# zacz08/ADM

Measured on AMD Instinct MI355X. Metric: train images/sec (CIFAR-10 32x32 uncond DDM UNet, 1 optimizer step/iter) + 10-step sample images/sec, higher is better.
Workload: dtype f32; 1 GPU; BASELINE configs[1]: CIFAR-10 32x32 uncond two-decoder DhariwalUNet (216M params), bs=128/GPU fp32, ddm_const schedule, dropout 0.1, loss_simple (LPIPS term needs unfetchable VGG16 weights), clip 1.0 + AdamW + EMA(every 8); global_batch=128, image=3x32x32, parallelism=dp1, valid=True

## Files before the change

### adm_amd/csrc/attention_h3.hip

```cpp
#include "common.h"
#include "split_format.h"

namespace {

constexpr int AH_KROW = 72;

__device__ __forceinline__ int ah_acc_row(int r, int lh) { return (r & 3) + 8 * (r >> 2) + 4 * lh; }
__device__ __forceinline__ int ah_pos16(int k) { return (((k >> 2) & 1) << 3) | ((k >> 3) << 2) | (k & 3); }

template <int NKT, bool MULTI>
__global__ __launch_bounds__(64 * NKT) void attn_fwd_h3_kernel(const float* __restrict__ qkv, float* __restrict__ out,
                                                                float* __restrict__ lse, int L, int heads,
                                                                const float* __restrict__ amax) {
  extern __shared__ __attribute__((aligned(16))) unsigned short smh[];
  constexpr int CH = NKT * 32;
  constexpr int VROW = CH + 8;
  unsigned short* Kh = smh;
  unsigned short* Vt = smh + 2 * CH * AH_KROW;
  const int tid = threadIdx.x, lane = tid & 63, wid = tid >> 6, lr = lane & 31, lh = lane >> 5;
  const int b = blockIdx.x / heads, h = blockIdx.x % heads;
  const long rs = (long)heads * 192;
  const float* base = qkv + (long)b * L * rs + h * 192;
  const float sc = split_scale(adm_amax_read(amax));
  const int q = (MULTI ? (int)blockIdx.y * CH : 0) + wid * 32 + lr;
  u32x4 q0[4], q1[4];
  {
    const float* qrow = base + (long)q * rs;
#pragma unroll
    for (int c = 0; c < 4; ++c) {
      const f32x4 lo = *reinterpret_cast<const f32x4*>(qrow + 16 * c + 8 * lh);
      const f32x4 hi = *reinterpret_cast<const f32x4*>(qrow + 16 * c + 8 * lh + 4);
      const float v[8] = {lo[0], lo[1], lo[2], lo[3], hi[0], hi[1], hi[2], hi[3]};
      split2_oct(v, sc * 0.125f, q0[c], q1[c]);
    }
  }
  const float inv_s = 1.f / (sc * sc);
  float m = -INFINITY, l = 0.f;
  f32x16 o[2];
#pragma unroll
  for (int r = 0; r < 16; ++r) { o[0][r] = 0.f; o[1][r] = 0.f; }
  const int nchunks = MULTI ? L / CH : 1;
#pragma unroll 1
  for (int kc = 0; kc < nchunks; ++kc) {
  const float* kbase = base + (long)kc * CH * rs;
  if (MULTI) __syncthreads();
  for (int i = tid; i < CH * 16; i += 64 * NKT) {
    const int key = i >> 4, c4 = i & 15;
    const f32x4 v = *reinterpret_cast<const f32x4*>(kbase + (long)key * rs + 64 + c4 * 4);
    unsigned t0[2], t1[2];
#pragma unroll
    for (int j = 0; j < 2; ++j) {
      const float x0 = v[2 * j] * sc, x1 = v[2 * j + 1] * sc;
      const _Float16 h00 = (_Float16)x0, h01 = (_Float16)x1;
      t0[j] = __builtin_bit_cast(unsigned, f16x2{h00, h01});
      t1[j] = __builtin_bit_cast(unsigned, f16x2{(_Float16)(x0 - (float)h00), (_Float16)(x1 - (float)h01)});
    }
    *reinterpret_cast<uint2*>(Kh + key * AH_KROW + c4 * 4) = make_uint2(t0[0], t0[1]);
    *reinterpret_cast<uint2*>(Kh + (CH + key) * AH_KROW + c4 * 4) = make_uint2(t1[0], t1[1]);
  }
  for (int i = tid; i < (CH / 2) * 16; i += 64 * NKT) {
    const int kp = i >> 4, c4 = i & 15;
    const int grp = kp >> 3, p0 = (kp & 7) * 2;
    const int k0 = grp * 16 + ((p0 & 7) & 3) + 8 * ((p0 & 7) >> 2) + 4 * (p0 >> 3);
    const f32x4 va = *reinterpret_cast<const f32x4*>(kbase + (long)k0 * rs + 128 + c4 * 4);
    const f32x4 vb = *reinterpret_cast<const f32x4*>(kbase + (long)(k0 + 1) * rs + 128 + c4 * 4);
#pragma unroll
    for (int j = 0; j < 4; ++j) {
      const float x0 = va[j] * sc, x1 = vb[j] * sc;
      const _Float16 h00 = (_Float16)x0, h01 = (_Float16)x1;
      const int d = c4 * 4 + j;
      *reinterpret_cast<unsigned*>(Vt + d * VROW + grp * 16 + p0) = __builtin_bit_cast(unsigned, f16x2{h00, h01});
      *reinterpret_cast<unsigned*>(Vt + (64 + d) * VROW + grp * 16 + p0) =
          __builtin_bit_cast(unsigned, f16x2{(_Float16)(x0 - (float)h00), (_Float16)(x1 - (float)h01)});
    }
  }
  __syncthreads();
  f32x16 s[NKT];
  float mc = -INFINITY;
#pragma unroll
  for (int kt = 0; kt < NKT; ++kt) {
    f32x16 acc;
#pragma unroll
    for (int r = 0; r < 16; ++r) acc[r] = 0.f;
    const unsigned short* krow = Kh + (kt * 32 + lr) * AH_KROW + 8 * lh;
#pragma unroll
    for (int c = 0; c < 4; ++c) {
      const f16x8 a0 = __builtin_bit_cast(f16x8, *reinterpret_cast<const u32x4*>(krow + 16 * c));
      const f16x8 a1 = __builtin_bit_cast(f16x8, *reinterpret_cast<const u32x4*>(krow + CH * AH_KROW + 16 * c));
      const f16x8 b0 = __builtin_bit_cast(f16x8, q0[c]), b1 = __builtin_bit_cast(f16x8, q1[c]);
      acc = __builtin_amdgcn_mfma_f32_32x32x16_f16(a0, b1, acc, 0, 0, 0);
      acc = __builtin_amdgcn_mfma_f32_32x32x16_f16(a1, b0, acc, 0, 0, 0);
      acc = __builtin_amdgcn_mfma_f32_32x32x16_f16(a0, b0, acc, 0, 0, 0);
    }
#pragma unroll
    for (int r = 0; r < 16; ++r) {
      s[kt][r] = acc[r] * inv_s;
      mc = fmaxf(mc, s[kt][r]);
    }
  }
  mc = fmaxf(mc, __shfl_xor(mc, 32, 64));
  const float mn = fmaxf(m, mc);
  if constexpr (MULTI) {
    const float rsc = (m == -INFINITY) ? 0.f : __expf(m - mn);
    l *= rsc;
#pragma unroll
    for (int r = 0; r < 16; ++r) { o[0][r] *= rsc; o[1][r] *= rsc; }
  }
#pragma unroll
  for (int kt = 0; kt < NKT; ++kt)
#pragma unroll
    for (int r = 0; r < 16; ++r) {
      const float e = __expf(s[kt][r] - mn);
      s[kt][r] = e;
      l += e;
    }
  m = mn;
#pragma unroll
  for (int kt = 0; kt < NKT; ++kt)
#pragma unroll
    for (int sl = 0; sl < 2; ++sl) {
      const float pv[8] = {s[kt][8 * sl], s[kt][8 * sl + 1], s[kt][8 * sl + 2], s[kt][8 * sl + 3],
                           s[kt][8 * sl + 4], s[kt][8 * sl + 5], s[kt][8 * sl + 6], s[kt][8 * sl + 7]};
      u32x4 p0, p1;
      split2_oct(pv, 16384.f, p0, p1);
      const f16x8 b0 = __builtin_bit_cast(f16x8, p0), b1 = __builtin_bit_cast(f16x8, p1);
#pragma unroll
      for (int db = 0; db < 2; ++db) {
        const unsigned short* vrow = Vt + (db * 32 + lr) * VROW + kt * 32 + 16 * sl + 8 * lh;
        const f16x8 a0 = __builtin_bit_cast(f16x8, *reinterpret_cast<const u32x4*>(vrow));
        const f16x8 a1 = __builtin_bit_cast(f16x8, *reinterpret_cast<const u32x4*>(vrow + 64 * VROW));
        o[db] = __builtin_amdgcn_mfma_f32_32x32x16_f16(a0, b1, o[db], 0, 0, 0);
        o[db] = __builtin_amdgcn_mfma_f32_32x32x16_f16(a1, b0, o[db], 0, 0, 0);
        o[db] = __builtin_amdgcn_mfma_f32_32x32x16_f16(a0, b0, o[db], 0, 0, 0);
      }
    }
  }
  const float mc = m;
  l += __shfl_xor(l, 32, 64);
  const float oscale = 1.f / (l * sc * 16384.f);
  float* orow = out + ((long)b * L + q) * heads * 64 + h * 64;
#pragma unroll
  for (int db = 0; db < 2; ++db)
#pragma unroll
    for (int q4 = 0; q4 < 4; ++q4) {
      const f32x4 v = {o[db][4 * q4] * oscale, o[db][4 * q4 + 1] * oscale, o[db][4 * q4 + 2] * oscale, o[db][4 * q4 + 3] * oscale};
      *reinterpret_cast<f32x4*>(orow + db * 32 + 8 * q4 + 4 * lh) = v;
    }
  if (lh == 0 && lse) lse[((long)b * heads + h) * L + q] = mc + __logf(l);
}

template <int NKT, bool MULTI>
int launch_fwd_h3(const float* qkv, float* out, float* lse, const float* amax, int B, int L, int heads, hipStream_t st) {
  constexpr int CH = NKT * 32;
  constexpr int smem = (2 * CH * AH_KROW + 2 * 64 * (CH + 8)) * (int)sizeof(unsigned short);
  static bool attr_set = false;
  if (!attr_set) {
    if (hipFuncSetAttribute(reinterpret_cast<const void*>(&attn_fwd_h3_kernel<NKT, MULTI>), hipFuncAttributeMaxDynamicSharedMemorySize, smem) != hipSuccess)
      return ADM_ELAUNCH;
    attr_set = true;
  }
  hipLaunchKernelGGL((attn_fwd_h3_kernel<NKT, MULTI>), dim3(B * heads, MULTI ? L / CH : 1), dim3(64 * NKT), smem, st, qkv, out, lse, L, heads, amax);
  ADM_CHECK_LAUNCH();
  return ADM_OK;
}

__device__ __forceinline__ f32x16 ah_mfma3(const u32x4 a0, const u32x4 a1, const u32x4 b0, const u32x4 b1, f32x16 c) {
  c = __builtin_amdgcn_mfma_f32_32x32x16_f16(__builtin_bit_cast(f16x8, a0), __builtin_bit_cast(f16x8, b1), c, 0, 0, 0);
  c = __builtin_amdgcn_mfma_f32_32x32x16_f16(__builtin_bit_cast(f16x8, a1), __builtin_bit_cast(f16x8, b0), c, 0, 0, 0);
  return __builtin_amdgcn_mfma_f32_32x32x16_f16(__builtin_bit_cast(f16x8, a0), __builtin_bit_cast(f16x8, b0), c, 0, 0, 0);
}
__device__ __forceinline__ void ah_fill_rows(unsigned short* dst, int CH, const float* src, long rs, float scale, int tid, int nthreads) {
  for (int i = tid; i < CH * 16; i += nthreads) {
    const int row = i >> 4, c4 = i & 15;
    const f32x4 v = *reinterpret_cast<const f32x4*>(src + (long)row * rs + c4 * 4);
    unsigned t0[2], t1[2];
#pragma unroll
    for (int j = 0; j < 2; ++j) {
      const float x0 = v[2 * j] * scale, x1 = v[2 * j + 1] * scale;
      const _Float16 h00 = (_Float16)x0, h01 = (_Float16)x1;
      t0[j] = __builtin_bit_cast(unsigned, f16x2{h00, h01});
      t1[j] = __builtin_bit_cast(unsigned, f16x2{(_Float16)(x0 - (float)h00), (_Float16)(x1 - (float)h01)});
    }
    *reinterpret_cast<uint2*>(dst + row * AH_KROW + c4 * 4) = make_uint2(t0[0], t0[1]);
    *reinterpret_cast<uint2*>(dst + (CH + row) * AH_KROW + c4 * 4) = make_uint2(t1[0], t1[1]);
  }
}
__device__ __forceinline__ void ah_fill_both(unsigned short* rimg, unsigned short* timg, int CH, const float* src, long rs, float scale,
                                             int tid, int nthreads) {
  const int VROW = CH + 8;
  for (int i = tid; i < (CH / 2) * 16; i += nthreads) {
    const int kp = i >> 4, c4 = i & 15;
    const int grp = kp >> 3, p0 = (kp & 7) * 2;
    const int r0 = grp * 16 + ((p0 & 7) & 3) + 8 * ((p0 & 7) >> 2) + 4 * (p0 >> 3);
    const f32x4 va = *reinterpret_cast<const f32x4*>(src + (long)r0 * rs + c4 * 4);
    const f32x4 vb = *reinterpret_cast<const f32x4*>(src + (long)(r0 + 1) * rs + c4 * 4);
    _Float16 a0[4], a1[4], b0[4], b1[4];
#pragma unroll
    for (int j = 0; j < 4; ++j) {
      const float x0 = va[j] * scale, x1 = vb[j] * scale;
      a0[j] = (_Float16)x0; a1[j] = (_Float16)(x0 - (float)a0[j]);
      b0[j] = (_Float16)x1; b1[j] = (_Float16)(x1 - (float)b0[j]);
      const int d = c4 * 4 + j;
      *reinterpret_cast<unsigned*>(timg + d * VROW + grp * 16 + p0) = __builtin_bit_cast(unsigned, f16x2{a0[j], b0[j]});
      *reinterpret_cast<unsigned*>(timg + (64 + d) * VROW + grp * 16 + p0) = __builtin_bit_cast(unsigned, f16x2{a1[j], b1[j]});
    }
    *reinterpret_cast<uint2*>(rimg + r0 * AH_KROW + c4 * 4) =
        make_uint2(__builtin_bit_cast(unsigned, f16x2{a0[0], a0[1]}), __builtin_bit_cast(unsigned, f16x2{a0[2], a0[3]}));
    *reinterpret_cast<uint2*>(rimg + (CH + r0) * AH_KROW + c4 * 4) =
        make_uint2(__builtin_bit_cast(unsigned, f16x2{a1[0], a1[1]}), __builtin_bit_cast(unsigned, f16x2{a1[2], a1[3]}));
    *reinterpret_cast<uint2*>(rimg + (r0 + 1) * AH_KROW + c4 * 4) =
        make_uint2(__builtin_bit_cast(unsigned, f16x2{b0[0], b0[1]}), __builtin_bit_cast(unsigned, f16x2{b0[2], b0[3]}));
    *reinterpret_cast<uint2*>(rimg + (CH + r0 + 1) * AH_KROW + c4 * 4) =
        make_uint2(__builtin_bit_cast(unsigned, f16x2{b1[0], b1[1]}), __builtin_bit_cast(unsigned, f16x2{b1[2], b1[3]}));
  }
}
__device__ __forceinline__ void ah_row_frag(const float* row, int lh, float scale, u32x4 (&t0)[4], u32x4 (&t1)[4]) {
#pragma unroll
  for (int c = 0; c < 4; ++c) {
    const f32x4 lo = *reinterpret_cast<const f32x4*>(row + 16 * c + 8 * lh);
    const f32x4 hi = *reinterpret_cast<const f32x4*>(row + 16 * c + 8 * lh + 4);
    const float v[8] = {lo[0], lo[1], lo[2], lo[3], hi[0], hi[1], hi[2], hi[3]};
    split2_oct(v, scale, t0[c], t1[c]);
  }
}
__device__ __forceinline__ f32x16 ah_rows_times_frag(const unsigned short* img, int CH, int row0, const u32x4 (&f0)[4], const u32x4 (&f1)[4],
                                                     int lr, int lh) {
  f32x16 acc;
#pragma unroll
  for (int r = 0; r < 16; ++r) acc[r] = 0.f;
  const unsigned short* rp = img + (row0 + lr) * AH_KROW + 8 * lh;
#pragma unroll
  for (int c = 0; c < 4; ++c)
    acc = ah_mfma3(*reinterpret_cast<const u32x4*>(rp + 16 * c), *reinterpret_cast<const u32x4*>(rp + CH * AH_KROW + 16 * c), f0[c], f1[c], acc);
  return acc;
}
__device__ __forceinline__ void ah_accum_T(f32x16 (&o)[2], const unsigned short* timg, int CH, int row0, const f32x16& t, float scale, int lr, int lh) {
  const int VROW = CH + 8;
#pragma unroll
  for (int sl = 0; sl < 2; ++sl) {
    const float tv[8] = {t[8 * sl], t[8 * sl + 1], t[8 * sl + 2], t[8 * sl + 3], t[8 * sl + 4], t[8 * sl + 5], t[8 * sl + 6], t[8 * sl + 7]};
    u32x4 b0, b1;
    split2_oct(tv, scale, b0, b1);
#pragma unroll
    for (int db = 0; db < 2; ++db) {
      const unsigned short* vp = timg + (db * 32 + lr) * VROW + row0 + 16 * sl + 8 * lh;
      o[db] = ah_mfma3(*reinterpret_cast<const u32x4*>(vp), *reinterpret_cast<const u32x4*>(vp + 64 * VROW), b0, b1, o[db]);
    }
  }
}
__device__ __forceinline__ void ah_store_T(const f32x16 (&o)[2], float* rowptr, int lh, float scale, float& am) {
#pragma unroll
  for (int db = 0; db < 2; ++db)
#pragma unroll
    for (int q4 = 0; q4 < 4; ++q4) {
      const f32x4 v = {o[db][4 * q4] * scale, o[db][4 * q4 + 1] * scale, o[db][4 * q4 + 2] * scale, o[db][4 * q4 + 3] * scale};
      am = fmaxf(fmaxf(am, fmaxf(fabsf(v[0]), fabsf(v[1]))), fmaxf(fabsf(v[2]), fabsf(v[3])));
      *reinterpret_cast<f32x4*>(rowptr + db * 32 + 8 * q4 + 4 * lh) = v;
    }
}

template <int NW>
__global__ __launch_bounds__(64 * NW) void attn_bwd_dq_h3_kernel(const float* __restrict__ qkv, const float* __restrict__ out,
                                                                   const float* __restrict__ dout, const float* __restrict__ lse,
                                                                   float* __restrict__ dqkv, float* __restrict__ delta, int L, int heads,
                                                                   const float* __restrict__ amax_qkv, const float* __restrict__ amax_g,
                                                                   float* __restrict__ amax_out) {
  extern __shared__ __attribute__((aligned(16))) unsigned short smh[];
  constexpr int CH = NW >= 4 ? 128 : 32 * NW;
  unsigned short* Kh = smh;
  unsigned short* Vh = Kh + 2 * CH * AH_KROW;
  unsigned short* Kt = Vh + 2 * CH * AH_KROW;
  const int tid = threadIdx.x, lane = tid & 63, wid = tid >> 6, lr = lane & 31, lh = lane >> 5;
  const int b = blockIdx.x / heads, h = blockIdx.x % heads;
  const long rs = (long)heads * 192, ro = (long)heads * 64;
  const float* base = qkv + (long)b * L * rs + h * 192;
  const float aq = adm_amax_read(amax_qkv), ag = adm_amax_read(amax_g);
  const float sc = split_scale(aq), sg = split_scale(ag), sd = split_scale(128.f * aq * ag);
  const int q = (int)blockIdx.y * 32 * NW + wid * 32 + lr;
  u32x4 q0[4], q1[4], g0[4], g1[4];
  ah_row_frag(base + (long)q * rs, lh, sc * 0.125f, q0, q1);
  const float* grow = dout + ((long)b * L + q) * ro + h * 64;
  const float* orow = out + ((long)b * L + q) * ro + h * 64;
  ah_row_frag(grow, lh, sg, g0, g1);
  float dl = 0.f;
#pragma unroll
  for (int c = 0; c < 4; ++c)
#pragma unroll
    for (int hh = 0; hh < 2; ++hh) {
      const f32x4 gv = *reinterpret_cast<const f32x4*>(grow + 16 * c + 8 * lh + 4 * hh);
      const f32x4 ov = *reinterpret_cast<const f32x4*>(orow + 16 * c + 8 * lh + 4 * hh);
      dl += gv[0] * ov[0] + gv[1] * ov[1] + gv[2] * ov[2] + gv[3] * ov[3];
    }
  dl += __shfl_xor(dl, 32, 64);
  const float ls = lse[((long)b * heads + h) * L + q];
  if (lh == 0) delta[((long)b * heads + h) * L + q] = dl;
  const float inv_s = 1.f / (sc * sc), inv_g = 1.f / (sc * sg);
  f32x16 dq[2];
#pragma unroll
  for (int r = 0; r < 16; ++r) { dq[0][r] = 0.f; dq[1][r] = 0.f; }
#pragma unroll 1
  for (int k0 = 0; k0 < L; k0 += CH) {
    __syncthreads();
    ah_fill_both(Kh, Kt, CH, base + (long)k0 * rs + 64, rs, sc, tid, 64 * NW);
    ah_fill_rows(Vh, CH, base + (long)k0 * rs + 128, rs, sc, tid, 64 * NW);
    __syncthreads();
#pragma unroll 1
    for (int kt = 0; kt < CH / 32; ++kt) {
      f32x16 s = ah_rows_times_frag(Kh, CH, kt * 32, q0, q1, lr, lh);
      const f32x16 dp = ah_rows_times_frag(Vh, CH, kt * 32, g0, g1, lr, lh);
#pragma unroll
      for (int r = 0; r < 16; ++r) s[r] = __expf(s[r] * inv_s - ls) * (dp[r] * inv_g - dl);
      ah_accum_T(dq, Kt, CH, kt * 32, s, sd, lr, lh);
    }
  }
  float am = 0.f;
  ah_store_T(dq, dqkv + ((long)b * L + q) * rs + h * 192, lh, 0.125f / (sc * sd), am);
  adm_amax_commit(am, amax_out);
}

template <int NW>
__global__ __launch_bounds__(64 * NW) void attn_bwd_dkv_h3_kernel(const float* __restrict__ qkv, const float* __restrict__ dout,
                                                                    const float* __restrict__ lse, const float* __restrict__ delta,
                                                                    float* __restrict__ dqkv, int L, int heads,
                                                                    const float* __restrict__ amax_qkv, const float* __restrict__ amax_g,
                                                                    float* __restrict__ amax_out) {
  extern __shared__ __attribute__((aligned(16))) unsigned short smh[];
  constexpr int CH = NW >= 4 ? 128 : 32 * NW;
  unsigned short* Qh = smh;
  unsigned short* Gh = Qh + 2 * CH * AH_KROW;
  unsigned short* Qt = Gh + 2 * CH * AH_KROW;
  unsigned short* Gt = Qt + 2 * 64 * (CH + 8);
  float* Ls = reinterpret_cast<float*>(Gt + 2 * 64 * (CH + 8));
  const int tid = threadIdx.x, lane = tid & 63, wid = tid >> 6, lr = lane & 31, lh = lane >> 5;
  const int b = blockIdx.x / heads, h = blockIdx.x % heads;
  const long rs = (long)heads * 192, ro = (long)heads * 64;
  const float* base = qkv + (long)b * L * rs + h * 192;
  const float aq = adm_amax_read(amax_qkv), ag = adm_amax_read(amax_g);
  const float sc = split_scale(aq), sg = split_scale(ag), sd = split_scale(128.f * aq * ag);
  const int key = (int)blockIdx.y * 32 * NW + wid * 32 + lr;
  u32x4 k0f[4], k1f[4], v0f[4], v1f[4];
  ah_row_frag(base + (long)key * rs + 64, lh, sc * 0.125f, k0f, k1f);
  ah_row_frag(base + (long)key * rs + 128, lh, sc, v0f, v1f);
  const float inv_s = 1.f / (sc * sc), inv_g = 1.f / (sg * sc);
  f32x16 dk[2], dv[2];
#pragma unroll
  for (int r = 0; r < 16; ++r) { dk[0][r] = 0.f; dk[1][r] = 0.f; dv[0][r] = 0.f; dv[1][r] = 0.f; }
#pragma unroll 1
  for (int q0 = 0; q0 < L; q0 += CH) {
    __syncthreads();
    const float* gsrc = dout + ((long)b * L + q0) * ro + h * 64;
    ah_fill_both(Qh, Qt, CH, base + (long)q0 * rs, rs, sc, tid, 64 * NW);
    ah_fill_both(Gh, Gt, CH, gsrc, ro, sg, tid, 64 * NW);
    for (int i = tid; i < CH; i += 64 * NW) {
      Ls[i] = lse[((long)b * heads + h) * L + q0 + i];
      Ls[CH + i] = delta[((long)b * heads + h) * L + q0 + i];
    }
    __syncthreads();
#pragma unroll 1
    for (int qt = 0; qt < CH / 32; ++qt) {
      f32x16 s = ah_rows_times_frag(Qh, CH, qt * 32, k0f, k1f, lr, lh);
      const f32x16 dp = ah_rows_times_frag(Gh, CH, qt * 32, v0f, v1f, lr, lh);
      f32x16 ds;
#pragma unroll
      for (int r = 0; r < 16; ++r) {
        const int qq = qt * 32 + ah_acc_row(r, lh);
        const float p = __expf(s[r] * inv_s - Ls[qq]);
        s[r] = p;
        ds[r] = p * (dp[r] * inv_g - Ls[CH + qq]);
      }
      ah_accum_T(dv, Gt, CH, qt * 32, s, 16384.f, lr, lh);
      ah_accum_T(dk, Qt, CH, qt * 32, ds, sd, lr, lh);
    }
  }
  float am = 0.f;
  float* orow = dqkv + ((long)b * L + key) * rs + h * 192;
  ah_store_T(dk, orow + 64, lh, 0.125f / (sc * sd), am);
  ah_store_T(dv, orow + 128, lh, 1.f / (sg * 16384.f), am);
  adm_amax_commit(am, amax_out);
}

template <int NW>
int launch_bwd_h3(const float* qkv, const float* out, const float* dout, const float* lse, float* dqkv, float* delta, const float* amax_qkv,
                  const float* amax_g, float* amax_out, int B, int L, int heads, hipStream_t st) {
  constexpr int CH = NW >= 4 ? 128 : 32 * NW;
  constexpr int smem_dq = (4 * CH * AH_KROW + 2 * 64 * (CH + 8)) * (int)sizeof(unsigned short);
  constexpr int smem_dkv = (4 * CH * AH_KROW + 4 * 64 * (CH + 8)) * (int)sizeof(unsigned short) + 2 * CH * (int)sizeof(float);
  static bool attr_set = false;
  if (!attr_set) {
    if (hipFuncSetAttribute(reinterpret_cast<const void*>(&attn_bwd_dq_h3_kernel<NW>), hipFuncAttributeMaxDynamicSharedMemorySize, smem_dq) != hipSuccess ||
        hipFuncSetAttribute(reinterpret_cast<const void*>(&attn_bwd_dkv_h3_kernel<NW>), hipFuncAttributeMaxDynamicSharedMemorySize, smem_dkv) != hipSuccess)
      return ADM_ELAUNCH;
    attr_set = true;
  }
  const dim3 grid(B * heads, L / (32 * NW));
  hipLaunchKernelGGL((attn_bwd_dq_h3_kernel<NW>), grid, dim3(64 * NW), smem_dq, st, qkv, out, dout, lse, dqkv, delta, L, heads,
                     amax_qkv, amax_g, amax_out);
  hipLaunchKernelGGL((attn_bwd_dkv_h3_kernel<NW>), grid, dim3(64 * NW), smem_dkv, st, qkv, dout, lse, delta, dqkv, L, heads,
                     amax_qkv, amax_g, amax_out);
  ADM_CHECK_LAUNCH();
  return ADM_OK;
}

}

extern "C" int adm_attn_bwd_h3(const float* qkv, const float* out, const float* dout, const float* lse, float* dqkv, float* delta,
                               const float* amax_qkv, const float* amax_dout, float* amax_dqkv, int B, int L, int heads, hipStream_t stream) {
  if (!qkv || !out || !dout || !lse || !dqkv || !delta || !amax_qkv || !amax_dout || B <= 0 || heads <= 0) return ADM_EINVAL;
  if (((uintptr_t)qkv | (uintptr_t)out | (uintptr_t)dout) & 15) return ADM_EINVAL;
  switch (L) {
    case 32: return launch_bwd_h3<1>(qkv, out, dout, lse, dqkv, delta, amax_qkv, amax_dout, amax_dqkv, B, L, heads, stream);
    case 64: return launch_bwd_h3<2>(qkv, out, dout, lse, dqkv, delta, amax_qkv, amax_dout, amax_dqkv, B, L, heads, stream);
    case 128: return launch_bwd_h3<4>(qkv, out, dout, lse, dqkv, delta, amax_qkv, amax_dout, amax_dqkv, B, L, heads, stream);
    case 256: return launch_bwd_h3<8>(qkv, out, dout, lse, dqkv, delta, amax_qkv, amax_dout, amax_dqkv, B, L, heads, stream);
    default:
      if (L > 256 && L % 256 == 0 && L <= 16384)
        return launch_bwd_h3<8>(qkv, out, dout, lse, dqkv, delta, amax_qkv, amax_dout, amax_dqkv, B, L, heads, stream);
      return ADM_EINVAL;
  }
}

extern "C" int adm_attn_fwd_h3(const float* qkv, float* out, float* lse, const float* amax, int B, int L, int heads, hipStream_t stream) {
  if (!qkv || !out || !amax || B <= 0 || heads <= 0 || ((uintptr_t)qkv & 15)) return ADM_EINVAL;
  switch (L) {
    case 32: return launch_fwd_h3<1, false>(qkv, out, lse, amax, B, L, heads, stream);
    case 64: return launch_fwd_h3<2, false>(qkv, out, lse, amax, B, L, heads, stream);
    case 128: return launch_fwd_h3<4, false>(qkv, out, lse, amax, B, L, heads, stream);
    case 256: return launch_fwd_h3<8, false>(qkv, out, lse, amax, B, L, heads, stream);
    default:
      if (L > 256 && L % 256 == 0 && L <= 16384) return launch_fwd_h3<8, true>(qkv, out, lse, amax, B, L, heads, stream);
      return ADM_EINVAL;
  }
}
```

Before: 1254 images/s.

## Hoist attention global loads ahead of amax read and prefetch next K/V chunk

The forward and dq-backward attention kernels now issue all Q/K/V (and dout/out) global loads into registers before waiting on the amax scale. A sched_barrier keeps that order, so memory latency overlaps the scale reduction. The amax is read per-lane from slotted copies and reduced with a wave max instead of through adm_amax_read. The dq kernel also prefetches the next K/V chunk into registers while the current one is computed, at the cost of higher register pressure and a new heads limit check.

```diff
diff --git a/adm_amd/csrc/attention_h3.hip b/adm_amd/csrc/attention_h3.hip
--- a/adm_amd/csrc/attention_h3.hip
+++ b/adm_amd/csrc/attention_h3.hip
@@ -7,6 +7,115 @@
 
 __device__ __forceinline__ int ah_acc_row(int r, int lh) { return (r & 3) + 8 * (r >> 2) + 4 * lh; }
 __device__ __forceinline__ int ah_pos16(int k) { return (((k >> 2) & 1) << 3) | ((k >> 3) << 2) | (k & 3); }
+
+__device__ __forceinline__ f32x4 ah_ld4(const float* p) { return *reinterpret_cast<const f32x4*>(p); }
+__device__ __forceinline__ f32x4 ah_ld4(const float* uni, unsigned boff) {
+  return *reinterpret_cast<const f32x4*>(reinterpret_cast<const char*>(uni) + boff);
+}
+__device__ __forceinline__ unsigned ah_opaque(unsigned boff) { asm volatile("" : "+v"(boff)); return boff; }
+constexpr int AH_MAX_HEADS = 16384;
+__device__ __forceinline__ float ah_amax_slot(const float* amax) { return amax[((threadIdx.x & 63) % ADM_AMAX_SLOTS) * ADM_AMAX_STRIDE]; }
+__device__ __forceinline__ float ah_wave_max(float v) {
+#pragma unroll
+  for (int o = 32; o > 0; o >>= 1) v = fmaxf(v, __shfl_xor(v, o, 64));
+  return v;
+}
+
+template <int NT>
+__device__ __forceinline__ f32x4 ah_row_ld(const float* src, long rs, int tid, int t) {
+  const unsigned boff = ah_opaque(((unsigned)(tid >> 4) * (unsigned)rs + (tid & 15) * 4) * 4u);
+  return ah_ld4(src + (long)(t * (NT / 16)) * rs, boff);
+}
+template <int CH, int NT>
+__device__ __forceinline__ void ah_row_st(unsigned short* dst, const f32x4 v, float scale, int tid, int t) {
+  const int i = tid + t * NT, row = i >> 4, c4 = i & 15;
+  unsigned t0[2], t1[2];
+#pragma unroll
+  for (int j = 0; j < 2; ++j) {
+    const float x0 = v[2 * j] * scale, x1 = v[2 * j + 1] * scale;
+    const _Float16 h00 = (_Float16)x0, h01 = (_Float16)x1;
+    t0[j] = __builtin_bit_cast(unsigned, f16x2{h00, h01});
+    t1[j] = __builtin_bit_cast(unsigned, f16x2{(_Float16)(x0 - (float)h00), (_Float16)(x1 - (float)h01)});
+  }
+  *reinterpret_cast<uint2*>(dst + row * AH_KROW + c4 * 4) = make_uint2(t0[0], t0[1]);
+  *reinterpret_cast<uint2*>(dst + (CH + row) * AH_KROW + c4 * 4) = make_uint2(t1[0], t1[1]);
+}
+__device__ __forceinline__ int ah_pair_row(int kp) {
+  const int grp = kp >> 3, p0 = (kp & 7) * 2;
+  return grp * 16 + ((p0 & 7) & 3) + 8 * ((p0 & 7) >> 2) + 4 * (p0 >> 3);
+}
+template <int NT>
+__device__ __forceinline__ void ah_pair_ld(f32x4& va, f32x4& vb, const float* src, long rs, int tid, int t) {
+  constexpr bool GROUPS = NT % 128 == 0;
+  const int r0 = ah_pair_row((tid >> 4) + (GROUPS ? 0 : t * (NT / 16)));
+  const unsigned boff = ah_opaque(((unsigned)r0 * (unsigned)rs + (tid & 15) * 4) * 4u);
+  const float* uni = src + (long)(GROUPS ? t * (NT / 8) : 0) * rs;
+  va = ah_ld4(uni, boff);
+  vb = ah_ld4(uni + rs, boff);
+}
+template <int CH, int NT, bool ROWS>
+__device__ __forceinline__ void ah_pair_st(unsigned short* rimg, unsigned short* timg, const f32x4 va, const f32x4 vb, float scale, int tid,
+                                           int t) {
+  constexpr int VROW = CH + 8;
+  const int i = tid + t * NT, kp = i >> 4, c4 = i & 15;
+  const int grp = kp >> 3, p0 = (kp & 7) * 2, r0 = ah_pair_row(kp);
+  _Float16 a0[4], a1[4], b0[4], b1[4];
+#pragma unroll
+  for (int j = 0; j < 4; ++j) {
+    const float x0 = va[j] * scale, x1 = vb[j] * scale;
+    a0[j] = (_Float16)x0; a1[j] = (_Float16)(x0 - (float)a0[j]);
+    b0[j] = (_Float16)x1; b1[j] = (_Float16)(x1 - (float)b0[j]);
+    const int d = c4 * 4 + j;
+    *reinterpret_cast<unsigned*>(timg + d * VROW + grp * 16 + p0) = __builtin_bit_cast(unsigned, f16x2{a0[j], b0[j]});
+    *reinterpret_cast<unsigned*>(timg + (64 + d) * VROW + grp * 16 + p0) = __builtin_bit_cast(unsigned, f16x2{a1[j], b1[j]});
+  }
+  if constexpr (ROWS) {
+    *reinterpret_cast<uint2*>(rimg + r0 * AH_KROW + c4 * 4) =
+        make_uint2(__builtin_bit_cast(unsigned, f16x2{a0[0], a0[1]}), __builtin_bit_cast(unsigned, f16x2{a0[2], a0[3]}));
+    *reinterpret_cast<uint2*>(rimg + (CH + r0) * AH_KROW + c4 * 4) =
+        make_uint2(__builtin_bit_cast(unsigned, f16x2{a1[0], a1[1]}), __builtin_bit_cast(unsigned, f16x2{a1[2], a1[3]}));
+    *reinterpret_cast<uint2*>(rimg + (r0 + 1) * AH_KROW + c4 * 4) =
+        make_uint2(__builtin_bit_cast(unsigned, f16x2{b0[0], b0[1]}), __builtin_bit_cast(unsigned, f16x2{b0[2], b0[3]}));
+    *reinterpret_cast<uint2*>(rimg + (CH + r0 + 1) * AH_KROW + c4 * 4) =
+        make_uint2(__builtin_bit_cast(unsigned, f16x2{b1[0], b1[1]}), __builtin_bit_cast(unsigned, f16x2{b1[2], b1[3]}));
+  }
+}
+template <int CH, int NT>
+__device__ __forceinline__ void ah_rows_load(f32x4 (&v)[CH * 16 / NT], const float* src, long rs, int tid) {
+#pragma unroll
+  for (int t = 0; t < CH * 16 / NT; ++t) v[t] = ah_row_ld<NT>(src, rs, tid, t);
+}
+template <int CH, int NT>
+__device__ __forceinline__ void ah_rows_store(unsigned short* dst, const f32x4 (&v)[CH * 16 / NT], float scale, int tid) {
+#pragma unroll
+  for (int t = 0; t < CH * 16 / NT; ++t) ah_row_st<CH, NT>(dst, v[t], scale, tid, t);
+}
+template <int CH, int NT>
+__device__ __forceinline__ void ah_pairs_load(f32x4 (&va)[CH * 8 / NT], f32x4 (&vb)[CH * 8 / NT], const float* src, long rs, int tid) {
+#pragma unroll
+  for (int t = 0; t < CH * 8 / NT; ++t) ah_pair_ld<NT>(va[t], vb[t], src, rs, tid, t);
+}
+template <int CH, int NT, bool ROWS>
+__device__ __forceinline__ void ah_pairs_store(unsigned short* rimg, unsigned short* timg, const f32x4 (&va)[CH * 8 / NT],
+                                               const f32x4 (&vb)[CH * 8 / NT], float scale, int tid) {
+#pragma unroll
+  for (int t = 0; t < CH * 8 / NT; ++t) ah_pair_st<CH, NT, ROWS>(rimg, timg, va[t], vb[t], scale, tid, t);
+}
+__device__ __forceinline__ void ah_frag_load(f32x4 (&r)[8], const float* row, int lh) {
+#pragma unroll
+  for (int c = 0; c < 4; ++c) {
+    r[2 * c] = ah_ld4(row + 16 * c + 8 * lh);
+    r[2 * c + 1] = ah_ld4(row + 16 * c + 8 * lh + 4);
+  }
+}
+__device__ __forceinline__ void ah_frag_split(const f32x4 (&r)[8], float scale, u32x4 (&t0)[4], u32x4 (&t1)[4]) {
+#pragma unroll
+  for (int c = 0; c < 4; ++c) {
+    const f32x4 lo = r[2 * c], hi = r[2 * c + 1];
+    const float v[8] = {lo[0], lo[1], lo[2], lo[3], hi[0], hi[1], hi[2], hi[3]};
+    split2_oct(v, scale, t0[c], t1[c]);
+  }
+}
 
 template <int NKT, bool MULTI>
 __global__ __launch_bounds__(64 * NKT) void attn_fwd_h3_kernel(const float* __restrict__ qkv, float* __restrict__ out,
@@ -21,58 +130,42 @@
   const int b = blockIdx.x / heads, h = blockIdx.x % heads;
   const long rs = (long)heads * 192;
   const float* base = qkv + (long)b * L * rs + h * 192;
-  const float sc = split_scale(adm_amax_read(amax));
+  const float araw = ah_amax_slot(amax);
   const int q = (MULTI ? (int)blockIdx.y * CH : 0) + wid * 32 + lr;
+  constexpr int NT = 64 * NKT;
+  f32x4 qr[8], kr[CH * 16 / NT], va[CH * 8 / NT], vb[CH * 8 / NT];
+  ah_frag_load(qr, base + (long)q * rs, lh);
+  if (!MULTI) {
+    ah_rows_load<CH, NT>(kr, base + 64, rs, tid);
+    ah_pairs_load<CH, NT>(va, vb, base + 128, rs, tid);
+  }
+  __builtin_amdgcn_sched_barrier(0);
+  const float sc = split_scale(ah_wave_max(araw));
   u32x4 q0[4], q1[4];
-  {
-    const float* qrow = base + (long)q * rs;
-#pragma unroll
-    for (int c = 0; c < 4; ++c) {
-      const f32x4 lo = *reinterpret_cast<const f32x4*>(qrow + 16 * c + 8 * lh);
-      const f32x4 hi = *reinterpret_cast<const f32x4*>(qrow + 16 * c + 8 * lh + 4);
-      const float v[8] = {lo[0], lo[1], lo[2], lo[3], hi[0], hi[1], hi[2], hi[3]};
-      split2_oct(v, sc * 0.125f, q0[c], q1[c]);
-    }
-  }
+  ah_frag_split(qr, sc * 0.125f, q0, q1);
   const float inv_s = 1.f / (sc * sc);
   float m = -INFINITY, l = 0.f;
   f32x16 o[2];
 #pragma unroll
   for (int r = 0; r < 16; ++r) { o[0][r] = 0.f; o[1][r] = 0.f; }
   const int nchunks = MULTI ? L / CH : 1;
-#pragma unroll 1
-  for (int kc = 0; kc < nchunks; ++kc) {
-  const float* kbase = base + (long)kc * CH * rs;
-  if (MULTI) __syncthreads();
-  for (int i = tid; i < CH * 16; i += 64 * NKT) {
-    const int key = i >> 4, c4 = i & 15;
-    const f32x4 v = *reinterpret_cast<const f32x4*>(kbase + (long)key * rs + 64 + c4 * 4);
-    unsigned t0[2], t1[2];
-#pragma unroll
-    for (int j = 0; j < 2; ++j) {
-      const float x0 = v[2 * j] * sc, x1 = v[2 * j + 1] * sc;
-      const _Float16 h00 = (_Float16)x0, h01 = (_Float16)x1;
-      t0[j] = __builtin_bit_cast(unsigned, f16x2{h00, h01});
-      t1[j] = __builtin_bit_cast(unsigned, f16x2{(_Float16)(x0 - (float)h00), (_Float16)(x1 - (float)h01)});
-    }
-    *reinterpret_cast<uint2*>(Kh + key * AH_KROW + c4 * 4) = make_uint2(t0[0], t0[1]);
-    *reinterpret_cast<uint2*>(Kh + (CH + key) * AH_KROW + c4 * 4) = make_uint2(t1[0], t1[1]);
-  }
-  for (int i = tid; i < (CH / 2) * 16; i += 64 * NKT) {
-    const int kp = i >> 4, c4 = i & 15;
-    const int grp = kp >> 3, p0 = (kp & 7) * 2;
-    const int k0 = grp * 16 + ((p0 & 7) & 3) + 8 * ((p0 & 7) >> 2) + 4 * (p0 >> 3);
-    const f32x4 va = *reinterpret_cast<const f32x4*>(kbase + (long)k0 * rs + 128 + c4 * 4);
-    const f32x4 vb = *reinterpret_cast<const f32x4*>(kbase + (long)(k0 + 1) * rs + 128 + c4 * 4);
-#pragma unroll
-    for (int j = 0; j < 4; ++j) {
-      const float x0 = va[j] * sc, x1 = vb[j] * sc;
-      const _Float16 h00 = (_Float16)x0, h01 = (_Float16)x1;
-      const int d = c4 * 4 + j;
-      *reinterpret_cast<unsigned*>(Vt + d * VROW + grp * 16 + p0) = __builtin_bit_cast(unsigned, f16x2{h00, h01});
-      *reinterpret_cast<unsigned*>(Vt + (64 + d) * VROW + grp * 16 + p0) =
-          __builtin_bit_cast(unsigned, f16x2{(_Float16)(x0 - (float)h00), (_Float16)(x1 - (float)h01)});
-    }
+  int kc = 0;
+#pragma unroll 1
+  for (;;) {
+  if constexpr (MULTI) {
+    const float* kbase = base + (long)kc * CH * rs;
+    __syncthreads();
+#pragma unroll 1
+    for (int t = 0; t < CH * 16 / NT; ++t) ah_row_st<CH, NT>(Kh, ah_row_ld<NT>(kbase + 64, rs, tid, t), sc, tid, t);
+#pragma unroll 1
+    for (int t = 0; t < CH * 8 / NT; ++t) {
+      f32x4 a, b;
+      ah_pair_ld<NT>(a, b, kbase + 128, rs, tid, t);
+      ah_pair_st<CH, NT, false>(nullptr, Vt, a, b, sc, tid, t);
+    }
+  } else {
+    ah_rows_store<CH, NT>(Kh, kr, sc, tid);
+    ah_pairs_store<CH, NT, false>(nullptr, Vt, va, vb, sc, tid);
   }
   __syncthreads();
   f32x16 s[NKT];
@@ -134,6 +227,7 @@
         o[db] = __builtin_amdgcn_mfma_f32_32x32x16_f16(a0, b0, o[db], 0, 0, 0);
       }
     }
+  if (!MULTI || ++kc == nchunks) break;
   }
   const float mc = m;
   l += __shfl_xor(l, 32, 64);
@@ -168,60 +262,6 @@
   c = __builtin_amdgcn_mfma_f32_32x32x16_f16(__builtin_bit_cast(f16x8, a0), __builtin_bit_cast(f16x8, b1), c, 0, 0, 0);
   c = __builtin_amdgcn_mfma_f32_32x32x16_f16(__builtin_bit_cast(f16x8, a1), __builtin_bit_cast(f16x8, b0), c, 0, 0, 0);
   return __builtin_amdgcn_mfma_f32_32x32x16_f16(__builtin_bit_cast(f16x8, a0), __builtin_bit_cast(f16x8, b0), c, 0, 0, 0);
-}
-__device__ __forceinline__ void ah_fill_rows(unsigned short* dst, int CH, const float* src, long rs, float scale, int tid, int nthreads) {
-  for (int i = tid; i < CH * 16; i += nthreads) {
-    const int row = i >> 4, c4 = i & 15;
-    const f32x4 v = *reinterpret_cast<const f32x4*>(src + (long)row * rs + c4 * 4);
-    unsigned t0[2], t1[2];
-#pragma unroll
-    for (int j = 0; j < 2; ++j) {
-      const float x0 = v[2 * j] * scale, x1 = v[2 * j + 1] * scale;
-      const _Float16 h00 = (_Float16)x0, h01 = (_Float16)x1;
-      t0[j] = __builtin_bit_cast(unsigned, f16x2{h00, h01});
-      t1[j] = __builtin_bit_cast(unsigned, f16x2{(_Float16)(x0 - (float)h00), (_Float16)(x1 - (float)h01)});
-    }
-    *reinterpret_cast<uint2*>(dst + row * AH_KROW + c4 * 4) = make_uint2(t0[0], t0[1]);
-    *reinterpret_cast<uint2*>(dst + (CH + row) * AH_KROW + c4 * 4) = make_uint2(t1[0], t1[1]);
-  }
-}
-__device__ __forceinline__ void ah_fill_both(unsigned short* rimg, unsigned short* timg, int CH, const float* src, long rs, float scale,
-                                             int tid, int nthreads) {
-  const int VROW = CH + 8;
-  for (int i = tid; i < (CH / 2) * 16; i += nthreads) {
-    const int kp = i >> 4, c4 = i & 15;
-    const int grp = kp >> 3, p0 = (kp & 7) * 2;
-    const int r0 = grp * 16 + ((p0 & 7) & 3) + 8 * ((p0 & 7) >> 2) + 4 * (p0 >> 3);
-    const f32x4 va = *reinterpret_cast<const f32x4*>(src + (long)r0 * rs + c4 * 4);
-    const f32x4 vb = *reinterpret_cast<const f32x4*>(src + (long)(r0 + 1) * rs + c4 * 4);
-    _Float16 a0[4], a1[4], b0[4], b1[4];
-#pragma unroll
-    for (int j = 0; j < 4; ++j) {
-      const float x0 = va[j] * scale, x1 = vb[j] * scale;
-      a0[j] = (_Float16)x0; a1[j] = (_Float16)(x0 - (float)a0[j]);
-      b0[j] = (_Float16)x1; b1[j] = (_Float16)(x1 - (float)b0[j]);
-      const int d = c4 * 4 + j;
-      *reinterpret_cast<unsigned*>(timg + d * VROW + grp * 16 + p0) = __builtin_bit_cast(unsigned, f16x2{a0[j], b0[j]});
-      *reinterpret_cast<unsigned*>(timg + (64 + d) * VROW + grp * 16 + p0) = __builtin_bit_cast(unsigned, f16x2{a1[j], b1[j]});
-    }
-    *reinterpret_cast<uint2*>(rimg + r0 * AH_KROW + c4 * 4) =
-        make_uint2(__builtin_bit_cast(unsigned, f16x2{a0[0], a0[1]}), __builtin_bit_cast(unsigned, f16x2{a0[2], a0[3]}));
-    *reinterpret_cast<uint2*>(rimg + (CH + r0) * AH_KROW + c4 * 4) =
-        make_uint2(__builtin_bit_cast(unsigned, f16x2{a1[0], a1[1]}), __builtin_bit_cast(unsigned, f16x2{a1[2], a1[3]}));
-    *reinterpret_cast<uint2*>(rimg + (r0 + 1) * AH_KROW + c4 * 4) =
-        make_uint2(__builtin_bit_cast(unsigned, f16x2{b0[0], b0[1]}), __builtin_bit_cast(unsigned, f16x2{b0[2], b0[3]}));
-    *reinterpret_cast<uint2*>(rimg + (CH + r0 + 1) * AH_KROW + c4 * 4) =
-        make_uint2(__builtin_bit_cast(unsigned, f16x2{b1[0], b1[1]}), __builtin_bit_cast(unsigned, f16x2{b1[2], b1[3]}));
-  }
-}
-__device__ __forceinline__ void ah_row_frag(const float* row, int lh, float scale, u32x4 (&t0)[4], u32x4 (&t1)[4]) {
-#pragma unroll
-  for (int c = 0; c < 4; ++c) {
-    const f32x4 lo = *reinterpret_cast<const f32x4*>(row + 16 * c + 8 * lh);
-    const f32x4 hi = *reinterpret_cast<const f32x4*>(row + 16 * c + 8 * lh + 4);
-    const float v[8] = {lo[0], lo[1], lo[2], lo[3], hi[0], hi[1], hi[2], hi[3]};
-    split2_oct(v, scale, t0[c], t1[c]);
-  }
 }
 __device__ __forceinline__ f32x16 ah_rows_times_frag(const unsigned short* img, int CH, int row0, const u32x4 (&f0)[4], const u32x4 (&f1)[4],
                                                      int lr, int lh) {
@@ -274,35 +314,39 @@
   const int b = blockIdx.x / heads, h = blockIdx.x % heads;
   const long rs = (long)heads * 192, ro = (long)heads * 64;
   const float* base = qkv + (long)b * L * rs + h * 192;
-  const float aq = adm_amax_read(amax_qkv), ag = adm_amax_read(amax_g);
+  const float aqraw = ah_amax_slot(amax_qkv), agraw = ah_amax_slot(amax_g);
+  const int q = (int)blockIdx.y * 32 * NW + wid * 32 + lr;
+  constexpr int NT = 64 * NW;
+  f32x4 qr[8], gr[8], orr[8], ka[CH * 8 / NT], kb[CH * 8 / NT], vr[CH * 16 / NT];
+  ah_frag_load(qr, base + (long)q * rs, lh);
+  ah_frag_load(gr, dout + ((long)b * L + q) * ro + h * 64, lh);
+  ah_frag_load(orr, out + ((long)b * L + q) * ro + h * 64, lh);
+  const float ls = lse[((long)b * heads + h) * L + q];
+  ah_pairs_load<CH, NT>(ka, kb, base + 64, rs, tid);
+  ah_rows_load<CH, NT>(vr, base + 128, rs, tid);
+  __builtin_amdgcn_sched_barrier(0);
+  const float aq = ah_wave_max(aqraw), ag = ah_wave_max(agraw);
   const float sc = split_scale(aq), sg = split_scale(ag), sd = split_scale(128.f * aq * ag);
-  const int q = (int)blockIdx.y * 32 * NW + wid * 32 + lr;
   u32x4 q0[4], q1[4], g0[4], g1[4];
-  ah_row_frag(base + (long)q * rs, lh, sc * 0.125f, q0, q1);
-  const float* grow = dout + ((long)b * L + q) * ro + h * 64;
-  const float* orow = out + ((long)b * L + q) * ro + h * 64;
-  ah_row_frag(grow, lh, sg, g0, g1);
+  ah_frag_split(qr, sc * 0.125f, q0, q1);
+  ah_frag_split(gr, sg, g0, g1);
   float dl = 0.f;
 #pragma unroll
-  for (int c = 0; c < 4; ++c)
-#pragma unroll
-    for (int hh = 0; hh < 2; ++hh) {
-      const f32x4 gv = *reinterpret_cast<const f32x4*>(grow + 16 * c + 8 * lh + 4 * hh);
-      const f32x4 ov = *reinterpret_cast<const f32x4*>(orow + 16 * c + 8 * lh + 4 * hh);
-      dl += gv[0] * ov[0] + gv[1] * ov[1] + gv[2] * ov[2] + gv[3] * ov[3];
-    }
+  for (int c = 0; c < 8; ++c) {
+    const f32x4 gv = gr[c], ov = orr[c];
+    dl += gv[0] * ov[0] + gv[1] * ov[1] + gv[2] * ov[2] + gv[3] * ov[3];
+  }
   dl += __shfl_xor(dl, 32, 64);
-  const float ls = lse[((long)b * heads + h) * L + q];
   if (lh == 0) delta[((long)b * heads + h) * L + q] = dl;
   const float inv_s = 1.f / (sc * sc), inv_g = 1.f / (sc * sg);
   f32x16 dq[2];
 #pragma unroll
   for (int r = 0; r < 16; ++r) { dq[0][r] = 0.f; dq[1][r] = 0.f; }
 #pragma unroll 1
-  for (int k0 = 0; k0 < L; k0 += CH) {
+  for (int k0 = 0;;) {
     __syncthreads();
-    ah_fill_both(Kh, Kt, CH, base + (long)k0 * rs + 64, rs, sc, tid, 64 * NW);
-    ah_fill_rows(Vh, CH, base + (long)k0 * rs + 128, rs, sc, tid, 64 * NW);
+    ah_pairs_store<CH, NT, true>(Kh, Kt, ka, kb, sc, tid);
+    ah_rows_store<CH, NT>(Vh, vr, sc, tid);
     __syncthreads();
 #pragma unroll 1
     for (int kt = 0; kt < CH / 32; ++kt) {
@@ -312,6 +356,9 @@
       for (int r = 0; r < 16; ++r) s[r] = __expf(s[r] * inv_s - ls) * (dp[r] * inv_g - dl);
       ah_accum_T(dq, Kt, CH, kt * 32, s, sd, lr, lh);
     }
+    if ((k0 += CH) >= L) break;
+    ah_pairs_load<CH, NT>(ka, kb, base + (long)k0 * rs + 64, rs, tid);
+    ah_rows_load<CH, NT>(vr, base + (long)k0 * rs + 128, rs, tid);
   }
   float am = 0.f;
   ah_store_T(dq, dqkv + ((long)b * L + q) * rs + h * 192, lh, 0.125f / (sc * sd), am);
@@ -338,9 +385,13 @@
   const float aq = adm_amax_read(amax_qkv), ag = adm_amax_read(amax_g);
   const float sc = split_scale(aq), sg = split_scale(ag), sd = split_scale(128.f * aq * ag);
   const int key = (int)blockIdx.y * 32 * NW + wid * 32 + lr;
+  constexpr int NT = 64 * NW;
+  f32x4 kr[8], vr[8];
+  ah_frag_load(kr, base + (long)key * rs + 64, lh);
+  ah_frag_load(vr, base + (long)key * rs + 128, lh);
   u32x4 k0f[4], k1f[4], v0f[4], v1f[4];
-  ah_row_frag(base + (long)key * rs + 64, lh, sc * 0.125f, k0f, k1f);
-  ah_row_frag(base + (long)key * rs + 128, lh, sc, v0f, v1f);
+  ah_frag_split(kr, sc * 0.125f, k0f, k1f);
+  ah_frag_split(vr, sc, v0f, v1f);
   const float inv_s = 1.f / (sc * sc), inv_g = 1.f / (sg * sc);
   f32x16 dk[2], dv[2];
 #pragma unroll
@@ -349,9 +400,19 @@
   for (int q0 = 0; q0 < L; q0 += CH) {
     __syncthreads();
     const float* gsrc = dout + ((long)b * L + q0) * ro + h * 64;
-    ah_fill_both(Qh, Qt, CH, base + (long)q0 * rs, rs, sc, tid, 64 * NW);
-    ah_fill_both(Gh, Gt, CH, gsrc, ro, sg, tid, 64 * NW);
-    for (int i = tid; i < CH; i += 64 * NW) {
+#pragma unroll 1
+    for (int t = 0; t < CH * 8 / NT; ++t) {
+      f32x4 a, c;
+      ah_pair_ld<NT>(a, c, base + (long)q0 * rs, rs, tid, t);
+      ah_pair_st<CH, NT, true>(Qh, Qt, a, c, sc, tid, t);
+    }
+#pragma unroll 1
+    for (int t = 0; t < CH * 8 / NT; ++t) {
+      f32x4 a, c;
+      ah_pair_ld<NT>(a, c, gsrc, ro, tid, t);
+      ah_pair_st<CH, NT, true>(Gh, Gt, a, c, sg, tid, t);
+    }
+    for (int i = tid; i < CH; i += NT) {
       Ls[i] = lse[((long)b * heads + h) * L + q0 + i];
       Ls[CH + i] = delta[((long)b * heads + h) * L + q0 + i];
     }
@@ -405,7 +466,7 @@
 
 extern "C" int adm_attn_bwd_h3(const float* qkv, const float* out, const float* dout, const float* lse, float* dqkv, float* delta,
                                const float* amax_qkv, const float* amax_dout, float* amax_dqkv, int B, int L, int heads, hipStream_t stream) {
-  if (!qkv || !out || !dout || !lse || !dqkv || !delta || !amax_qkv || !amax_dout || B <= 0 || heads <= 0) return ADM_EINVAL;
+  if (!qkv || !out || !dout || !lse || !dqkv || !delta || !amax_qkv || !amax_dout || B <= 0 || heads <= 0 || heads > AH_MAX_HEADS) return ADM_EINVAL;
   if (((uintptr_t)qkv | (uintptr_t)out | (uintptr_t)dout) & 15) return ADM_EINVAL;
   switch (L) {
     case 32: return launch_bwd_h3<1>(qkv, out, dout, lse, dqkv, delta, amax_qkv, amax_dout, amax_dqkv, B, L, heads, stream);
@@ -420,7 +481,7 @@
 }
 
 extern "C" int adm_attn_fwd_h3(const float* qkv, float* out, float* lse, const float* amax, int B, int L, int heads, hipStream_t stream) {
-  if (!qkv || !out || !amax || B <= 0 || heads <= 0 || ((uintptr_t)qkv & 15)) return ADM_EINVAL;
+  if (!qkv || !out || !amax || B <= 0 || heads <= 0 || heads > AH_MAX_HEADS || ((uintptr_t)qkv & 15)) return ADM_EINVAL;
   switch (L) {
     case 32: return launch_fwd_h3<1, false>(qkv, out, lse, amax, B, L, heads, stream);
     case 64: return launch_fwd_h3<2, false>(qkv, out, lse, amax, B, L, heads, stream);
```

Result: no change. 1258 images/s (median of 6 runs) (+0.3%).
